# aleju/cat-generator

Hardware: AMD Instinct MI355X
Metric: images/sec per G+D step, G32up-c 32x32 RGB bs=128 per GPU (higher is better)
Workload: dtype f32

## Files before the change

### cat-generator_amd/csrc/common.h

```cpp
#pragma once
#include <hip/hip_runtime.h>
#include <algorithm>
#include <stdint.h>
#include <stdio.h>
#include <string.h>
#include "../../include/catgan.h"

namespace cg {

char* err_buf();
int fail(const char* fmt, ...);

inline hipStream_t S(void* s) { return reinterpret_cast<hipStream_t>(s); }

#define CG_HIP(call)                                                              \
    do {                                                                          \
        hipError_t e__ = (call);                                                  \
        if (e__ != hipSuccess)                                                    \
            return cg::fail("%s:%d %s -> %s", __FILE__, __LINE__, #call,          \
                            hipGetErrorString(e__));                              \
    } while (0)

#define CG_LAUNCH_CHECK()                                                         \
    do {                                                                          \
        hipError_t e__ = hipGetLastError();                                       \
        if (e__ != hipSuccess)                                                    \
            return cg::fail("%s:%d kernel launch -> %s", __FILE__, __LINE__,      \
                            hipGetErrorString(e__));                              \
    } while (0)

#define CG_REQUIRE(cond, ...)                                                     \
    do {                                                                          \
        if (!(cond)) return cg::fail(__VA_ARGS__);                                \
    } while (0)

constexpr int kNumCU = 256;

#ifndef CG_TIMING_PROBE
#define CG_TIMING_PROBE 0
#endif
#define CG_PROBE_HALF(fam, T) (((CG_TIMING_PROBE) & (fam)) ? ((T) + 1) / 2 : (T))
constexpr int kEwWgsPerCU = 4, kColReduceWgsPerCU = 1;

enum Opt {
    OPT_SKINNY, OPT_GEMM_BK32, OPT_WINO_BK, OPT_NN_TILE, OPT_TN_TILE, OPT_NN_SPLITS, OPT_TN_SPLITS,
    OPT_XCD_SWIZZLE, OPT_NN_GLDS, OPT_TN_GLDS, OPT_WINO_GLDS, OPT_PAD_SKIP, OPT_WINO3, OPT_WINO_DGRAD_FUSE, OPT_WINO_DGRAD_FUSE_LAUNCHES,
    OPT_WINO3_LAUNCHES, OPT_PACK_WIDE, OPT_SAMPLER_ATOMIC_LAUNCHES, OPT_COUNT
};
long opt(Opt o);
void opt_count(Opt o);

static inline int cdiv(long a, long b) { return (int)((a + b - 1) / b); }

constexpr size_t kColScratchBytes = 8u << 20;
void* col_scratch(hipStream_t stream);
hipStream_t queue_stream(hipStream_t ref, int cls, int slot);
int queue_class(hipStream_t ref, hipStream_t s);

constexpr int MAXG = 4;
constexpr int kMaxStridedGroups = 36;
template <typename T>
__device__ __forceinline__ T sel4(int i, T a, T b, T c, T d) { return i == 0 ? a : (i == 1 ? b : (i == 2 ? c : d)); }
__device__ __forceinline__ float4 ld4(const float* p) { return *reinterpret_cast<const float4*>(p); }
__device__ __forceinline__ float f4c(const float4& v, int i) { return i == 0 ? v.x : (i == 1 ? v.y : (i == 2 ? v.z : v.w)); }
template <typename T>
static inline void set4(T& p0, T& p1, T& p2, T& p3, const T* src, int n) {
    T* const dst[MAXG] = {&p0, &p1, &p2, &p3};
    for (int i = 0; i < MAXG; ++i) *dst[i] = (src && i < n) ? src[i] : nullptr;
}
__device__ __host__ __forceinline__ int phase_map(int a, int d, int pad) { return ((a + d - pad) >> 1) - ((a - pad) >> 1); }
static inline int phase_kp(int k, int pad) { return phase_map(0, k - 1, pad) + 1; }

struct WgradParts {
    const float* part;
    const float* bias_part;
    float* const* gw;
    float* const* gb;
    long gws;
    int ngroups, S, Cin, Cout, kH, kW, pad, ups;
    float scale;
};
int wgrad_finish(hipStream_t st, const WgradParts& w, bool defer);
void wgrad_discard_all();

constexpr int kSkinnyWgradBlocks = 512;
bool skinny_ok(int ngroups, int Cin, int Cout, int kH, int kW, int padH, int padW, int ups);
size_t skinny_wgrad_ws_bytes(int Cin, int Cout);
void skinny_valu_forward(hipStream_t st, const float* x, const float* w, const float* bias, float* y, int N, int H, int W, int Cin, int Cout);
void skinny_valu_wgrad(hipStream_t st, const float* x, const float* dy, float* part, float* bias_part, int N, int H, int W, int Cin, int Cout,
                       int blocks, long ppb);
bool skinny_mfma_ok(int Cin, int Cout, int H, int W);
int skinny_mfma_forward(hipStream_t st, const float* x, const float* w, const float* bias, float* y, int N, int H, int W, int Cin, int Cout);
int skinny_mfma_wgrad(hipStream_t st, const float* x, const float* dy, float* part, float* bias_part, int N, int H, int W, int Cin, int Cout,
                      int max_blocks);

bool head_wgrad_ok(int N, int T, int C, int Co);
int head_wgrad(hipStream_t st, const float* x, const float* dy, float* gw, float* gb, int N, int T, int C, int Co, float scale);
constexpr int kWino3UOffset = 9 * 64 * 64, kWino3UFloats = 16 * 64 * 64;
static inline bool wino3_layer(int Cout, int Cin, int kH, int kW) { return Cout == 64 && Cin == 64 && kH == 3 && kW == 3; }
bool wino3_geom_ok(int ngroups, int N, int H, int W, int Cin, int Cout, int kH, int kW, int padH, int padW, int ups);
int wino3_note_pack(hipStream_t st, int n, const float* const* w, float* const* wf, float* const* wb, const int* Cout, const int* Cin,
                    const int* kH, const int* kW, const int* wb_map);
int wino3_forward(hipStream_t st, int ngroups, const float* const* x, const float* const* wpk, const float* const* bias, float* const* y,
                  int N, int H, int W);

static inline int ew_grid(long n, int per_block = 256) {
    long b = (n + per_block - 1) / per_block;
    if (b < 1) b = 1;
    const long cap = (long)kNumCU * kEwWgsPerCU;
    if (b > cap) b = cap;
    return (int)b;
}

static inline bool al16(const void* p) { return ((uintptr_t)p & 15) == 0; }
template <class... P>
static inline bool vec_ok(long n, const P*... p) { return n % 4 == 0 && (al16(p) && ...); }

constexpr int tile_of_row_c(int l) {
    return ((l < 4 || (l >= 12 && l < 16) || (l >= 20 && l < 28)) ? 0 : 16) +
           ((l < 4 || (l >= 12 && l < 16) || (l >= 20 && l < 28)) ? (l < 4 ? l : (l < 16 ? l - 8 : l - 12)) : (l < 12 ? l - 4 : (l < 20 ? l - 8 : l - 16)));
}
__device__ __forceinline__ int tile_of_row(int l) {
    const bool ga = l < 4 || (l >= 12 && l < 16) || (l >= 20 && l < 28);
    const int rank = ga ? (l < 4 ? l : (l < 16 ? l - 8 : l - 12)) : (l < 12 ? l - 4 : (l < 20 ? l - 8 : l - 16));
    return (ga ? 0 : 16) + rank;
}
__device__ __forceinline__ void wino3_pack_item(const float* __restrict__ w, float* uf, float* ub, int idx) {
    constexpr int C = 64;
    const int co = idx / C, ci = idx % C;
    const float G[4][3] = {{1.f, 0.f, 0.f}, {.5f, .5f, .5f}, {.5f, -.5f, .5f}, {0.f, 0.f, 1.f}};
    for (int flip = 0; flip < 2; ++flip) {
        float* U = flip ? ub : uf;
        if (!U) continue;
        float g[3][3];
        for (int a = 0; a < 3; ++a)
            for (int b = 0; b < 3; ++b) g[a][b] = flip ? w[((long)ci * C + co) * 9 + (2 - a) * 3 + (2 - b)] : w[((long)co * C + ci) * 9 + a * 3 + b];
        float t[4][3];
        for (int i = 0; i < 4; ++i)
            for (int b = 0; b < 3; ++b) t[i][b] = G[i][0] * g[0][b] + G[i][1] * g[1][b] + G[i][2] * g[2][b];
        for (int i = 0; i < 4; ++i)
            for (int k = 0; k < 4; ++k)
                U[(((long)(i * 4 + k) * (C / 4) + ci / 4) * C + co) * 4 + (ci & 3)] = t[i][0] * G[k][0] + t[i][1] * G[k][1] + t[i][2] * G[k][2];
    }
}
__device__ __forceinline__ float u01(uint64_t seed, uint64_t ctr) {
    uint64_t z = seed + (ctr + 1) * 0x9E3779B97F4A7C15ull;
    z = (z ^ (z >> 30)) * 0xBF58476D1CE4E5B9ull;
    z = (z ^ (z >> 27)) * 0x94D049BB133111EBull;
    z = z ^ (z >> 31);
    return (float)(z >> 40) * (1.0f / 16777216.0f);
}
__device__ __forceinline__ float wave_sum(float v) {
#pragma unroll
    for (int off = 32; off > 0; off >>= 1) v += __shfl_down(v, off, 64);
    return v;
}
__device__ __forceinline__ double wave_sum(double v) {
#pragma unroll
    for (int off = 32; off > 0; off >>= 1) v += __shfl_down(v, off, 64);
    return v;
}

#ifndef CG_COL_HANDOVER
#define CG_COL_HANDOVER 3
#endif
__device__ __forceinline__ void st_agent(double* p, double v) {
#if CG_COL_HANDOVER == 4
    const unsigned long long old = __hip_atomic_exchange((unsigned long long*)p, (unsigned long long)__double_as_longlong(v),
                                                         __ATOMIC_RELAXED, __HIP_MEMORY_SCOPE_AGENT);
    asm volatile("" ::"v"(old));
#else
    __hip_atomic_store(p, v, __ATOMIC_RELAXED, __HIP_MEMORY_SCOPE_AGENT);
#endif
}
__device__ __forceinline__ double ld_agent(const double* p) {
#if CG_COL_HANDOVER == 4
    unsigned long long zero = 0ull;
    asm volatile("" : "+v"(zero));
    return __longlong_as_double((long long)__hip_atomic_fetch_or((unsigned long long*)const_cast<double*>(p), zero, __ATOMIC_RELAXED,
                                                                 __HIP_MEMORY_SCOPE_AGENT));
#else
    return __hip_atomic_load(const_cast<double*>(p), __ATOMIC_RELAXED, __HIP_MEMORY_SCOPE_AGENT);
#endif
}

__device__ __forceinline__ bool last_block_arrives(unsigned* counter, unsigned total) {
    __shared__ int last_flag;
#if CG_COL_HANDOVER == 0
    __threadfence();
#else
    asm volatile("s_waitcnt vmcnt(0)" ::: "memory");
#endif
    __syncthreads();
    if (threadIdx.x == 0) {
#if CG_COL_HANDOVER == 3
        __builtin_amdgcn_fence(__ATOMIC_RELEASE, "agent");
#endif
        const unsigned t = __hip_atomic_fetch_add(counter, 1u, __ATOMIC_RELAXED, __HIP_MEMORY_SCOPE_AGENT);
        last_flag = (t == total - 1) ? 1 : 0;
        if (last_flag) __hip_atomic_store(counter, 0u, __ATOMIC_RELAXED, __HIP_MEMORY_SCOPE_AGENT);
    }
    __syncthreads();
#if CG_COL_HANDOVER == 0
    if (last_flag) __threadfence();
#elif CG_COL_HANDOVER == 3
    if (last_flag) __builtin_amdgcn_fence(__ATOMIC_ACQUIRE, "agent");
#endif
    return last_flag != 0;
}

struct ColTree {
    int G, ngroups;
    unsigned* counters;
    double* part;
    double* grp;
    double* extra;
};
constexpr int kColTreeMaxGroups = 32;
static inline bool col_tree_layout(char* scr, long chunks, size_t nk, size_t nextra, ColTree& t) {
    t.G = (int)std::max<long>(16, (chunks + kColTreeMaxGroups - 1) / kColTreeMaxGroups);
    t.ngroups = (int)((chunks + t.G - 1) / t.G);
    t.counters = (unsigned*)scr;
    t.part = (double*)(scr + 256);
    t.grp = t.part + (size_t)chunks * nk;
    t.extra = t.grp + (size_t)t.ngroups * nk;
    return 256 + sizeof(double) * ((size_t)chunks * nk + (size_t)t.ngroups * nk + nextra) <= kColScratchBytes;
}

__device__ __forceinline__ void col_sum_rows(const double* rows, int nrows, int nk, double* out) {
    for (int k = threadIdx.x; k < nk; k += blockDim.x) {
        double t = 0.0;
        int y = 0;
        for (; y + 16 <= nrows; y += 16) {
            double v[16];
#pragma unroll
            for (int j = 0; j < 16; ++j) v[j] = ld_agent(&rows[(size_t)(y + j) * nk + k]);
#pragma unroll
            for (int j = 0; j < 16; ++j) t += v[j];
        }
        for (; y < nrows; ++y) t += ld_agent(&rows[(size_t)y * nk + k]);
        st_agent(&out[k], t);
    }
}

__device__ __forceinline__ bool col_tree_finish(const ColTree& t, int chunk, int chunks, unsigned blocks_per_chunk, int nk, double* sums) {
    const int g = chunk / t.G;
    const int in_group = min(t.G, chunks - g * t.G);
    if (!last_block_arrives(t.counters + 1 + g, (unsigned)in_group * blocks_per_chunk)) return false;
    col_sum_rows(t.part + (size_t)g * t.G * nk, in_group, nk, t.grp + (size_t)g * nk);
    if (!last_block_arrives(t.counters, (unsigned)t.ngroups)) return false;
    col_sum_rows(t.grp, t.ngroups, nk, sums);
    return true;
}

__device__ __forceinline__ double block_sum_256(double v, double* sh ) {
    v = wave_sum(v);
    const int lane = threadIdx.x & 63, wave = threadIdx.x >> 6;
    if (lane == 0) sh[wave] = v;
    __syncthreads();
    double r = 0.0;
    if (threadIdx.x == 0) r = sh[0] + sh[1] + sh[2] + sh[3];
    __syncthreads();
    return r;
}

#define CG_GRID_STRIDE(i, n) \
    for (long i = blockIdx.x * (long)blockDim.x + threadIdx.x; i < (n); i += (long)gridDim.x * blockDim.x)

template <int VW> struct Vec;
template <> struct Vec<1> {
    typedef float T;
    static __device__ __forceinline__ T zero() { return 0.f; }
    static __device__ __forceinline__ T ld(const float* p) { return *p; }
    static __device__ __forceinline__ void st(float* p, T v) { *p = v; }
    static __device__ __forceinline__ float dot(T a, T b) { return a * b; }
    static __device__ __forceinline__ void fma(T& acc, float w, T g) { acc += w * g; }
    T v;
    __device__ __forceinline__ float& operator[](int) { return v; }
    __device__ __forceinline__ float operator[](int) const { return v; }
    static __device__ __forceinline__ Vec load(const float* p, long i) { return Vec{p[i]}; }
    __device__ __forceinline__ void store(float* p, long i) const { p[i] = v; }
    static __device__ __forceinline__ Vec ldc(const float* p, int c) { return Vec{p[c]}; }
};
template <> struct Vec<4> {
    typedef float4 T;
    static __device__ __forceinline__ T zero() { return make_float4(0.f, 0.f, 0.f, 0.f); }
    static __device__ __forceinline__ T ld(const float* p) { return *reinterpret_cast<const float4*>(p); }
    static __device__ __forceinline__ void st(float* p, T v) { *reinterpret_cast<float4*>(p) = v; }
    static __device__ __forceinline__ float dot(T a, T b) { return ((a.x * b.x + a.y * b.y) + a.z * b.z) + a.w * b.w; }
    static __device__ __forceinline__ void fma(T& acc, float w, T g) { acc.x += w * g.x; acc.y += w * g.y; acc.z += w * g.z; acc.w += w * g.w; }
    T v;
    __device__ __forceinline__ float& operator[](int k) { return (&v.x)[k]; }
    __device__ __forceinline__ float operator[](int k) const { return (&v.x)[k]; }
    static __device__ __forceinline__ Vec load(const float* p, long i) { return Vec{ld(p + 4 * i)}; }
    __device__ __forceinline__ void store(float* p, long i) const { st(p + 4 * i, v); }
    static __device__ __forceinline__ Vec ldc(const float* p, int c) { return Vec{make_float4(p[4 * c], p[4 * c + 1], p[4 * c + 2], p[4 * c + 3])}; }
};

__device__ __forceinline__ bool act_passes(int act, float x) { return act == 0 || (act == 1 ? x > 0.f : x >= 0.f); }
__device__ __forceinline__ float act(int act, float v, float a) { return act_passes(act, v) ? v : a * v; }
__device__ __forceinline__ float dact(int act, float x, float d, float a) { return act_passes(act, x) ? d : a * d; }
__device__ __forceinline__ float slope_term(float x, float d) { return x <= 0.f ? x * d : 0.f; }
template <int VW>
__device__ __forceinline__ void slope_acc(float& s, const Vec<VW>& x, const Vec<VW>& d) {
    if constexpr (VW == 1) {
        if (x[0] <= 0.f) s = fmaf(x[0], d[0], s);
    } else {
        float t = slope_term(x[0], d[0]);
#pragma unroll
        for (int k = 1; k < VW; ++k) t += slope_term(x[k], d[k]);
        s += t;
    }
}
template <int VW>
__device__ __forceinline__ void prelu_bwd_walk(const float* x, const float* dy, float a, float* dx, long n, double* partial) {
    __shared__ double sh[4];
    float s = 0.f;
    CG_GRID_STRIDE(i, n) {
        const Vec<VW> v = Vec<VW>::load(x, i), g = Vec<VW>::load(dy, i);
        Vec<VW> o;
#pragma unroll
        for (int k = 0; k < VW; ++k) o[k] = dact(1, v[k], g[k], a);
        o.store(dx, i);
        slope_acc(s, v, g);
    }
    if (!partial) return;
    const double t = block_sum_256((double)s, sh);
    if (threadIdx.x == 0) *partial = t;
}
__device__ __forceinline__ double partials_sum_256(const double* part, int nparts) {
    __shared__ double sh[4];
    double s = 0.0;
    for (int i = threadIdx.x; i < nparts; i += 256) s += part[i];
    return block_sum_256(s, sh);
}
__device__ __forceinline__ float bn_xhat(float x, float m, float s) { return (x - m) * s; }
__device__ __forceinline__ float bn_norm(float x, float m, float s, float g, float b) { return bn_xhat(x, m, s) * g + b; }
__device__ __forceinline__ float bn_dx(float x, float dy, float g, float m, float s, float m1, float m2) {
    return g * s * (dy - m1 - bn_xhat(x, m, s) * m2);
}
__device__ __forceinline__ float augment_noise(uint64_t seed, uint64_t ctr) {
    unsigned S = 0;
#pragma unroll
    for (int k = 0; k < 3; ++k) {
        uint64_t z = seed + (ctr + k + 1) * 0x9E3779B97F4A7C15ull;
        z = (z ^ (z >> 30)) * 0xBF58476D1CE4E5B9ull;
        z = (z ^ (z >> 27)) * 0x94D049BB133111EBull;
        z = z ^ (z >> 31);
        S += (unsigned)(z & 0xFFFF) + (unsigned)((z >> 16) & 0xFFFF) + (unsigned)((z >> 32) & 0xFFFF) + (unsigned)(z >> 48);
    }
// ... 13 lines not shown
```

### cat-generator_amd/csrc/ops.hip

```cpp
#include "common.h"
#include <stdarg.h>
#include <stdlib.h>
#include <algorithm>

namespace cg {
char* err_buf() {
    static thread_local char buf[512] = {0};
    return buf;
}
int fail(const char* fmt, ...) {
    va_list ap;
    va_start(ap, fmt);
    vsnprintf(err_buf(), 512, fmt, ap);
    va_end(ap);
    return 1;
}

namespace {
struct OptDef { const char* name; long dflt; };
const OptDef kOptDefs[OPT_COUNT] = {
    {"CG_SKINNY", 1}, {"CG_GEMM_BK32", 1}, {"CG_WINO_BK", 0}, {"CG_NN_TILE", 0}, {"CG_TN_TILE", 0}, {"CG_NN_SPLITS", 0}, {"CG_TN_SPLITS", 0},
    {"CG_XCD_SWIZZLE", 7}, {"CG_NN_GLDS", 1}, {"CG_TN_GLDS", 1}, {"CG_WINO_GLDS", 1}, {"CG_PAD_SKIP", 20}, {"CG_WINO3", 1},
    {"CG_WINO_DGRAD_FUSE", 1}, {"CG_WINO_DGRAD_FUSE_LAUNCHES", 0}, {"CG_WINO3_LAUNCHES", 0}, {"CG_PACK_WIDE", 1},
    {"CG_SAMPLER_ATOMIC_LAUNCHES", 0},
};
long g_opt_val[OPT_COUNT];
int g_opt_state[OPT_COUNT];
}

}
#include <chrono>
#include <mutex>
#include <unordered_map>
#include <vector>
namespace cg {
void* col_scratch(hipStream_t stream) {
    constexpr int kPool = 8, kReserve = 4;
    static std::unordered_map<hipStream_t, void*> blocks;
    static std::vector<void*> pool;
    static std::mutex mu;
    std::lock_guard<std::mutex> lk(mu);
    auto it = blocks.find(stream);
    if (it != blocks.end()) return it->second;
    hipStreamCaptureStatus st = hipStreamCaptureStatusNone;
    const bool capturing = stream && hipStreamIsCapturing(stream, &st) == hipSuccess && st != hipStreamCaptureStatusNone;
    if (capturing && pool.empty()) {
        cg::fail("column reduce: no scratch block left for a stream first used inside a graph capture (run one pass on it before cg_graph_begin)");
        return nullptr;
    }
    if (!capturing && (int)pool.size() <= kReserve) {
        char* p = nullptr;
        hipStreamCaptureMode mode = hipStreamCaptureModeRelaxed;
        (void)hipThreadExchangeStreamCaptureMode(&mode);
        const bool ok = hipMalloc((void**)&p, kColScratchBytes * kPool) == hipSuccess &&
                        hipMemsetAsync(p, 0, kColScratchBytes * kPool, stream) == hipSuccess &&
                        hipStreamSynchronize(stream) == hipSuccess;
        (void)hipThreadExchangeStreamCaptureMode(&mode);
        if (!ok) {
            (void)hipGetLastError();
            if (pool.empty()) { cg::fail("column reduce: cannot allocate %zu bytes of scratch", kColScratchBytes * kPool); return nullptr; }
        } else
            for (int i = kPool - 1; i >= 0; --i) pool.insert(pool.begin(), p + (size_t)i * kColScratchBytes);
    }
    void* blk = pool.back();
    pool.pop_back();
    blocks[stream] = blk;
    return blk;
}
namespace {
__global__ void queue_probe_spin_k(unsigned long long ticks, int* sink) {
    const unsigned long long t0 = wall_clock64();
    while (wall_clock64() - t0 < ticks) { }
    if (ticks == ~0ull) *sink = 1;
}
struct QueuePool {
    std::vector<hipStream_t> s;
    std::unordered_map<hipStream_t, std::vector<int>> cls;
    std::mutex mu;
};
QueuePool& qpool() { static QueuePool p; return p; }
constexpr int kQueuePool = 24;

double probe_pair(hipStream_t a, hipStream_t b, bool both, unsigned long long ticks) {
    (void)hipStreamSynchronize(a);
    if (both) (void)hipStreamSynchronize(b);
    const auto t0 = std::chrono::steady_clock::now();
    hipLaunchKernelGGL(queue_probe_spin_k, dim3(1), dim3(64), 0, a, ticks, (int*)nullptr);
    if (both) hipLaunchKernelGGL(queue_probe_spin_k, dim3(1), dim3(64), 0, b, ticks, (int*)nullptr);
    (void)hipStreamSynchronize(a);
    if (both) (void)hipStreamSynchronize(b);
    return std::chrono::duration<double, std::milli>(std::chrono::steady_clock::now() - t0).count();
}
bool same_queue(hipStream_t a, hipStream_t b) {
    const unsigned long long ticks = 30000;
    int votes = 0;
    for (int r = 0; r < 3; ++r) {
        const double one = probe_pair(a, a, false, ticks), two = probe_pair(a, b, true, ticks);
        if (two > 1.6 * one) ++votes;
    }
    return votes >= 2;
}
}

int queue_classify(hipStream_t ref) {
    QueuePool& p = qpool();
    hipStreamCaptureStatus st = hipStreamCaptureStatusNone;
    if (ref && hipStreamIsCapturing(ref, &st) == hipSuccess && st != hipStreamCaptureStatusNone)
        return cg::fail("queue_stream: a stream's hardware queue cannot be probed inside a graph capture (run one pass on it before cg_graph_begin)");
    while ((int)p.s.size() < kQueuePool) {
        hipStream_t q;
        if (hipStreamCreateWithFlags(&q, hipStreamNonBlocking) != hipSuccess) return cg::fail("queue_stream: hipStreamCreate failed");
        p.s.push_back(q);
    }
    std::vector<int> c(p.s.size(), -1);
    std::vector<hipStream_t> rep;
    for (size_t i = 0; i < p.s.size(); ++i) {
        if (same_queue(ref, p.s[i])) { c[i] = 0; continue; }
        for (size_t k = 0; k < rep.size() && c[i] < 0; ++k)
            if (same_queue(rep[k], p.s[i])) c[i] = (int)k + 1;
        if (c[i] < 0) { rep.push_back(p.s[i]); c[i] = (int)rep.size(); }
    }
    (void)hipGetLastError();
    p.cls[ref] = c;
    return 0;
}

hipStream_t queue_stream(hipStream_t ref, int cls, int slot) {
    QueuePool& p = qpool();
    std::lock_guard<std::mutex> lk(p.mu);
    if (!p.cls.count(ref) && queue_classify(ref)) return nullptr;
    const std::vector<int>& c = p.cls[ref];
    int nclass = 0;
    for (int v : c) nclass = std::max(nclass, v + 1);
    if (nclass < 2) {
        static bool warned = false;
        if (!warned) { warned = true; fprintf(stderr, "cg: the hardware-queue probe found one queue only - side streams are plain pool streams (overlap not guaranteed)\n"); }
        return p.s[(size_t)((cls & 3) * (kQueuePool / 4) + slot % (kQueuePool / 4)) % p.s.size()];
    }
    cls = cls % nclass;
    int seen = 0;
    hipStream_t last = nullptr;
    for (size_t i = 0; i < c.size(); ++i)
        if (c[i] == cls) { last = p.s[i]; if (seen++ == slot) return p.s[i]; }
    if (last) return last;
    cg::fail("queue_stream: no pool stream on hardware queue class %d", cls);
    return nullptr;
}

int queue_class(hipStream_t ref, hipStream_t s) {
    if (s == ref) return 0;
    QueuePool& p = qpool();
    std::lock_guard<std::mutex> lk(p.mu);
    auto it = p.cls.find(ref);
    if (it == p.cls.end()) return -1;
    for (size_t i = 0; i < p.s.size(); ++i) if (p.s[i] == s) return it->second[i];
    return -1;
}

unsigned long g_opt_epoch = 1;
long opt(Opt o) {
    if (g_opt_state[o] == 0) {
        const char* e = getenv(kOptDefs[o].name);
        g_opt_val[o] = e ? atol(e) : kOptDefs[o].dflt;
        g_opt_state[o] = 1;
    }
    return g_opt_val[o];
}
void opt_count(Opt o) { opt(o); ++g_opt_val[o]; }
}

namespace {
using cg::block_sum_256;
using cg::last_block_arrives;
using cg::wave_sum;

#define GRID_STRIDE(i, n) CG_GRID_STRIDE(i, n)

enum { CS_RGB = 0, CS_Y = 1, CS_YUV = 2, CS_HSL = 3 };
__device__ __forceinline__ void store_colorspace(float* dst, long i, float r, float g, float b, int cs) {
#pragma clang fp contract(off)
    if (cs == CS_RGB) { dst[3 * i] = r; dst[3 * i + 1] = g; dst[3 * i + 2] = b; }
    else if (cs == CS_Y) {
        const float t0 = 0.21f * r, t1 = 0.72f * g, t2 = 0.07f * b;
        dst[i] = (t0 + t1) + t2;
    } else if (cs == CS_YUV) {
        const float y0 = 0.299f * r, y1 = 0.587f * g, y2 = 0.114f * b;
        const float u0 = -0.14713f * r, u1 = 0.28886f * g, u2 = 0.436f * b;
        const float v0 = 0.615f * r, v1 = 0.51499f * g, v2 = 0.10001f * b;
        dst[3 * i] = (y0 + y1) + y2; dst[3 * i + 1] = (u0 - u1) + u2; dst[3 * i + 2] = (v0 - v1) - v2;
    } else {
        const float mx = fmaxf(r, fmaxf(g, b)), mn = fminf(r, fminf(g, b));
        const float sum = mx + mn, l = __fdiv_rn(sum, 2.f);
        float h = 0.f, s = 0.f;
        if (mx != mn) {
            const float d = mx - mn;
            s = l > 0.5f ? __fdiv_rn(d, (2.f - mx) - mn) : __fdiv_rn(d, sum);
            if (mx == r) h = __fdiv_rn(g - b, d) + (g < b ? 6.f : 0.f);
            else if (mx == g) h = __fdiv_rn(b - r, d) + 2.f;
            else h = __fdiv_rn(r - g, d) + 4.f;
            h = __fdiv_rn(h, 6.f);
        }
        dst[3 * i] = h; dst[3 * i + 1] = s; dst[3 * i + 2] = l;
    }
}
__device__ __forceinline__ float hsl_hue(float p, float q, float t) {
#pragma clang fp contract(off)
    const float sixth = (float)(1.0 / 6.0), two_thirds = (float)(2.0 / 3.0);
    if (t < 0.f) t += 1.f;
    if (t > 1.f) t -= 1.f;
    if (t < sixth) { const float a = (q - p) * 6.f, m = a * t; return p + m; }
    if (t < 0.5f) return q;
    if (t < two_thirds) { const float a = (q - p) * (two_thirds - t), m = a * 6.f; return p + m; }
    return p;
}
__device__ __forceinline__ void colorspace_to_rgb(float a, float b, float c, int cs, float* rgb) {
#pragma clang fp contract(off)
    if (cs == CS_YUV) {
        const float rv = 1.13983f * c, gu = 0.39465f * b, gv = 0.58060f * c, bu = 2.03211f * b;
        rgb[0] = a + rv; rgb[1] = (a - gu) - gv; rgb[2] = a + bu;
    } else {
        const float h = a, s = b, l = c;
        if (s == 0.f) { rgb[0] = l; rgb[1] = l; rgb[2] = l; return; }
        const float third = (float)(1.0 / 3.0);
        const float ls = l * s;
        const float q = l < 0.5f ? l * (1.f + s) : (l + s) - ls;
        const float p = 2.f * l - q;
        rgb[0] = hsl_hue(p, q, h + third); rgb[1] = hsl_hue(p, q, h); rgb[2] = hsl_hue(p, q, h - third);
    }
}
__global__ void colorspace_convert_k(const float* src, float* dst, long npix, int from, int to) {
    GRID_STRIDE(i, npix) {
        const float a = src[3 * i], b = src[3 * i + 1], c = src[3 * i + 2];
        if (from == CS_RGB) store_colorspace(dst, i, a, b, c, to);
        else {
            float rgb[3];
            colorspace_to_rgb(a, b, c, from, rgb);
            dst[3 * i] = rgb[0]; dst[3 * i + 1] = rgb[1]; dst[3 * i + 2] = rgb[2];
        }
    }
}
__global__ void images_u8_to_f32_k(const unsigned char* __restrict__ src, float* __restrict__ dst, long npix, int cs) {
#pragma clang fp contract(off)
    GRID_STRIDE(i, npix) {
        const float r = __fdiv_rn((float)src[3 * i], 255.f), g = __fdiv_rn((float)src[3 * i + 1], 255.f), b = __fdiv_rn((float)src[3 * i + 2], 255.f);
        store_colorspace(dst, i, r, g, b, cs);
    }
}

__device__ __forceinline__ float scale_axis(const float* w, int base, int Ls, int Ld, int d) {
#pragma clang fp contract(off)
#define s(k) w[(k) - base]
    if (Ld == Ls) return s(d);
    if (Ld > Ls) {
        if (d == Ld - 1 || Ls == 1) return s(Ls == 1 ? 0 : Ls - 1);
        const float scale = __fdiv_rn((float)(Ls - 1), (float)(Ld - 1));
        float sf = (float)d * scale;
        const int si = (int)sf;
        sf -= (float)si;
        const float a = (1.f - sf) * s(si), b = sf * s(si + 1);
        return a + b;
    }
    const float scale = __fdiv_rn((float)Ls, (float)Ld);
    float f0 = (float)d * scale;
    int i0 = (int)f0;
    f0 -= (float)i0;
    if (d == 0) { i0 = 0; f0 = 0.f; }
    float f1 = (float)(d + 1) * scale;
    const int i1 = (int)f1;
    f1 -= (float)i1;
    float acc = (1.f - f0) * s(i0), n = 1.f - f0;
    for (int si = i0 + 1; si < i1; ++si) { acc += s(si); n += 1.f; }
    if (i1 < Ls) { const float t = f1 * s(i1); acc += t; n += f1; }
    return __fdiv_rn(acc, n);
#undef s
}
__device__ __forceinline__ void scale_pixel(const unsigned char* __restrict__ im, float* __restrict__ dst, long i, int ox, int oy, int Hs, int Ws,
                                            int Hd, int Wd, int cs) {
#pragma clang fp contract(off)
    int y0 = oy, y1 = oy;
    if (Hd < Hs) {
        const float scale = __fdiv_rn((float)Hs, (float)Hd);
        y0 = oy == 0 ? 0 : (int)((float)oy * scale);
        y1 = min(Hs - 1, (int)((float)(oy + 1) * scale));
    } else if (Hd > Hs) {
        const float scale = __fdiv_rn((float)(Hs - 1), (float)(Hd - 1));
        y0 = (oy == Hd - 1 || Hs == 1) ? Hs - 1 : (int)((float)oy * scale);
        y1 = min(Hs - 1, y0 + 1);
    }
    float rgb[3];
    for (int c = 0; c < 3; ++c) {
        float col[8];
        for (int y = y0; y <= y1 && y - y0 < 8; ++y) {
            int x0 = ox, x1 = ox;
            if (Wd < Ws) {
                const float sc = __fdiv_rn((float)Ws, (float)Wd);
                x0 = ox == 0 ? 0 : (int)((float)ox * sc);
                x1 = min(Ws - 1, (int)((float)(ox + 1) * sc));
            } else if (Wd > Ws) {
                const float sc = __fdiv_rn((float)(Ws - 1), (float)(Wd - 1));
                x0 = (ox == Wd - 1 || Ws == 1) ? Ws - 1 : (int)((float)ox * sc);
                x1 = min(Ws - 1, x0 + 1);
            }
            float row[8];
            for (int x = x0; x <= x1 && x - x0 < 8; ++x) row[x - x0] = __fdiv_rn((float)im[((long)y * Ws + x) * 3 + c], 255.f);
            col[y - y0] = scale_axis(row, x0, Ws, Wd, ox);
        }
        rgb[c] = scale_axis(col, y0, Hs, Hd, oy);
    }
    store_colorspace(dst, i, rgb[0], rgb[1], rgb[2], cs);
}
__device__ __forceinline__ void store_zero_pixel(float* dst, long i, int cs) {
    if (cs == CS_Y) dst[i] = 0.f;
    else { dst[3 * i] = 0.f; dst[3 * i + 1] = 0.f; dst[3 * i + 2] = 0.f; }
}
__global__ void images_u8_scale_k(const unsigned char* __restrict__ src, float* __restrict__ dst, int N, int Hs, int Ws, int Hd, int Wd, int cs) {
    const long total = (long)N * Hd * Wd;
    GRID_STRIDE(i, total) {
        const int ox = (int)(i % Wd), oy = (int)((i / Wd) % Hd);
        const long n = i / ((long)Wd * Hd);
        scale_pixel(src + n * (long)Hs * Ws * 3, dst, i, ox, oy, Hs, Ws, Hd, Wd, cs);
    }
}
__global__ void images_u8_gather_scale_k(const unsigned char* __restrict__ set, long M, const int32_t* __restrict__ idx, float* __restrict__ dst,
                                         int N, int Hs, int Ws, int Hd, int Wd, int cs) {
    const long total = (long)N * Hd * Wd;
    GRID_STRIDE(i, total) {
        const int ox = (int)(i % Wd), oy = (int)((i / Wd) % Hd);
// ... 1605 lines not shown
```

### cat-generator_amd/csrc/wino3.hip

```cpp
#include "common.h"

namespace {

typedef float f32x16 __attribute__((ext_vector_type(16)));
typedef unsigned int u32x4 __attribute__((ext_vector_type(4)));
typedef float f32x4 __attribute__((ext_vector_type(4)));
constexpr int C = 64;
constexpr int PLD = 68;
constexpr int PW = 18, PH = 10;
constexpr int kUFloats = cg::kWino3UFloats;

using cg::ld4;
__device__ __forceinline__ float4 bufld4(__amdgpu_buffer_rsrc_t r, unsigned voff, int soff) {
    const u32x4 v = __builtin_amdgcn_raw_buffer_load_b128(r, voff, soff, 0);
    const f32x4 f = __builtin_bit_cast(f32x4, v);
    return make_float4(f.x, f.y, f.z, f.w);
}

struct PackJobs { const float* w[8]; float* uf[8]; float* ub[8]; int n; };
__global__ void wino3_pack_k(PackJobs jobs) {
    cg::wino3_pack_item(jobs.w[blockIdx.y], jobs.uf[blockIdx.y], jobs.ub[blockIdx.y], blockIdx.x * 256 + threadIdx.x);
}

using cg::tile_of_row;
using cg::tile_of_row_c;

template <int XI>
__device__ __forceinline__ void wino_row(const float* P, int tyl, int txl, int h, __amdgpu_buffer_rsrc_t rsU, unsigned uvoff, f32x16 (&T)[2]) {
    constexpr int I1 = XI == 0 ? 0 : (XI == 2 ? 2 : 1), I2 = XI == 0 ? 2 : (XI == 1 ? 2 : (XI == 2 ? 1 : 3));
    constexpr bool PLUS = XI == 1;
    const float* pt = P + ((2 * tyl) * PW + 2 * txl) * PLD;
    const float* r1 = pt + I1 * PW * PLD + ((h ^ ((tyl + (I1 >> 1)) & 1)) << 2);
    const float* r2 = pt + I2 * PW * PLD + ((h ^ ((tyl + (I2 >> 1)) & 1)) << 2);
    f32x16 acc[4];
#pragma unroll
    for (int k = 0; k < 4; ++k)
#pragma unroll
        for (int r = 0; r < 16; ++r) acc[k][r] = 0.f;
#pragma unroll 2
    for (int s = 0; s < CG_PROBE_HALF(8, 8); ++s) {
        float4 e[4];
#pragma unroll
        for (int c = 0; c < 4; ++c) {
            const float4 d1 = ld4(r1 + c * PLD + 8 * s), d2 = ld4(r2 + c * PLD + 8 * s);
            e[c].x = PLUS ? d1.x + d2.x : d1.x - d2.x; e[c].y = PLUS ? d1.y + d2.y : d1.y - d2.y;
            e[c].z = PLUS ? d1.z + d2.z : d1.z - d2.z; e[c].w = PLUS ? d1.w + d2.w : d1.w - d2.w;
        }
        float4 v[4], ua[4];
#pragma unroll
        for (int nu = 0; nu < 4; ++nu) {
            constexpr int J1[4] = {0, 1, 2, 1}, J2[4] = {2, 2, 1, 3};
            const float4 a = e[J1[nu]], b = e[J2[nu]];
            if (nu == 1) { v[nu].x = a.x + b.x; v[nu].y = a.y + b.y; v[nu].z = a.z + b.z; v[nu].w = a.w + b.w; }
            else { v[nu].x = a.x - b.x; v[nu].y = a.y - b.y; v[nu].z = a.z - b.z; v[nu].w = a.w - b.w; }
            ua[nu] = bufld4(rsU, uvoff, (((XI * 4 + nu) * 16 + 2 * s) * C) * 16);
        }
#define CG_W3_MF(comp) \
    _Pragma("unroll") for (int nu = 0; nu < 4; ++nu) acc[nu] = __builtin_amdgcn_mfma_f32_32x32x2f32(v[nu].comp, ua[nu].comp, acc[nu], 0, 0, 0);
        CG_W3_MF(x) CG_W3_MF(y) CG_W3_MF(z) CG_W3_MF(w)
#undef CG_W3_MF
    }
#pragma unroll
    for (int r = 0; r < 16; ++r) { T[0][r] = (acc[0][r] + acc[1][r]) + acc[2][r]; T[1][r] = (acc[1][r] - acc[2][r]) - acc[3][r]; }
}

struct W3Args {
    const float* x[4]; const float* u[4]; const float* bias[4]; float* y[4];
    int N, H, W;
};

__global__ __launch_bounds__(512, 2) void wino3_fused_k(W3Args a) {
    __shared__ __attribute__((aligned(16))) float P[PH * PW * PLD];
    const int tid = threadIdx.x, lane = tid & 63, wave = __builtin_amdgcn_readfirstlane(tid >> 6);
    const int j = lane & 31, h = lane >> 5;
    const int xi = wave & 3, nt = wave >> 2;
    const int grp = blockIdx.y;
    const float* __restrict__ x = a.x[grp];
    const float* __restrict__ U = a.u[grp];
    float* __restrict__ y = a.y[grp];
    const int H = a.H, W = a.W;
    const int bxn = W >> 4, byn = H >> 3;
    int b = blockIdx.x;
    const int bx = b % bxn; b /= bxn;
    const int by = b % byn;
    const int n = b / byn;
    const int y0 = by * 8, x0 = bx * 16;

    {
        const __amdgpu_buffer_rsrc_t rsx = __builtin_amdgcn_make_buffer_rsrc((void*)(x + (long)n * H * W * C), 0, (unsigned)(H * W * C * 4), 0x00020000);
        const int q = tid & 15;
        int pix = tid >> 4, pr = pix / PW, pc = pix - pr * PW;
#pragma unroll
        for (int it = 0; it < (PH * PW + 31) / 32; ++it) {
            const int iy = y0 - 1 + pr, ix = x0 - 1 + pc;
            const bool in = iy >= 0 && iy < H && ix >= 0 && ix < W;
            const unsigned voff = in ? (unsigned)(((iy * W + ix) * C + q * 4) * 4) : 0x80000000u;
            const float4 v = bufld4(rsx, voff, 0);
            if (pix < PH * PW) *reinterpret_cast<float4*>(P + pix * PLD + ((q ^ ((pr >> 1) & 1)) << 2)) = v;
            pix += 32; pr += 1; pc += 14;
            if (pc >= PW) { pc -= PW; pr += 1; }
        }
    }
    __syncthreads();

    const int tl = tile_of_row(j), tyl = tl >> 3, txl = tl & 7;
    const __amdgpu_buffer_rsrc_t rsU = __builtin_amdgcn_make_buffer_rsrc((void*)U, 0, kUFloats * 4, 0x00020000);
    const unsigned uvoff = (unsigned)(h * C + nt * 32 + j) * 16u;
    f32x16 T[2];
    if (xi == 0) wino_row<0>(P, tyl, txl, h, rsU, uvoff, T);
    else if (xi == 1) wino_row<1>(P, tyl, txl, h, rsU, uvoff, T);
    else if (xi == 2) wino_row<2>(P, tyl, txl, h, rsU, uvoff, T);
    else wino_row<3>(P, tyl, txl, h, rsU, uvoff, T);

    __syncthreads();
    float* X = P + nt * 6 * 1024;
#pragma unroll
    for (int r = 0; r < 16; ++r) {
        const int k = r * 64 + lane;
        if (xi == 1) { X[0 * 1024 + k] = T[0][r]; X[5 * 1024 + k] = T[1][r]; }
        if (xi == 2) { X[1 * 1024 + k] = T[0][r]; X[3 * 1024 + k] = T[1][r]; }
        if (xi == 0) X[2 * 1024 + k] = T[1][r];
        if (xi == 3) X[4 * 1024 + k] = T[0][r];
    }
    __syncthreads();
    const int oa = xi >> 1, ob = xi & 1;
    const float* bias = a.bias[grp];
    const float bco = bias ? bias[nt * 32 + j] : 0.f;
    const __amdgpu_buffer_rsrc_t rsy = __builtin_amdgcn_make_buffer_rsrc((void*)(y + (long)n * H * W * C), 0, (unsigned)(H * W * C * 4), 0x00020000);
    const int lane_base = (((y0 + oa) * W + x0 + ob) * C + nt * 32 + j) * 4;
    const int rowb = 2 * W * C * 4, colb = 2 * C * 4;
#pragma unroll
    for (int r = 0; r < 16; ++r) {
        const int k = r * 64 + lane;
        float v;
        if (xi == 0) v = (T[0][r] + X[0 * 1024 + k]) + X[1 * 1024 + k];
        else if (xi == 1) v = (X[2 * 1024 + k] + T[1][r]) + X[3 * 1024 + k];
        else if (xi == 2) v = (X[0 * 1024 + k] - T[0][r]) - X[4 * 1024 + k];
        else v = (X[5 * 1024 + k] - X[3 * 1024 + k]) - T[1][r];
        const int row0 = (r & 3) + 8 * (r >> 2);
        const int t0 = tile_of_row_c(row0), t1 = tile_of_row_c(row0 + 4);
        const int off0 = (t0 >> 3) * rowb + (t0 & 7) * colb, off1 = (t1 >> 3) * rowb + (t1 & 7) * colb;
        __builtin_amdgcn_raw_buffer_store_b32(__float_as_uint(v + bco), rsy, lane_base + (h ? off1 : off0), 0, 0);
    }
}

}

namespace cg {

bool wino3_geom_ok(int ngroups, int N, int H, int W, int Cin, int Cout, int kH, int kW, int padH, int padW, int ups) {
    if (!(ups == 0 && kH == 3 && kW == 3 && padH == 1 && padW == 1 && Cin == C && Cout == C && H % 8 == 0 && W % 16 == 0)) return false;
    if (ngroups < 1 || ngroups > 4) return false;
    const long v = opt(OPT_WINO3);
    const bool full = (long)ngroups * N * (H / 8) * (W / 16) >= 2L * kNumCU;
    return v == 2 || (v == 1 && full);
}

int wino3_note_pack(hipStream_t st, int n, const float* const* w, float* const* wf, float* const* wb, const int* Cout, const int* Cin,
                    const int* kH, const int* kW, const int* wb_map) {
    PackJobs jobs;
    jobs.n = 0;
    auto flush = [&]() {
        if (jobs.n) hipLaunchKernelGGL(wino3_pack_k, dim3(C * C / 256, jobs.n), dim3(256), 0, st, jobs);
        jobs.n = 0;
    };
    for (int i = 0; i < n; ++i) {
        if (!wino3_layer(Cout[i], Cin[i], kH[i], kW[i]) || (wb_map && wb_map[i])) continue;
        jobs.w[jobs.n] = w[i];
        jobs.uf[jobs.n] = wf[i] ? wf[i] + kWino3UOffset : nullptr;
        jobs.ub[jobs.n] = wb[i] ? wb[i] + kWino3UOffset : nullptr;
        if (++jobs.n == 8) flush();
    }
    flush();
    CG_LAUNCH_CHECK();
    return 0;
}

int wino3_forward(hipStream_t st, int ngroups, const float* const* x, const float* const* wpk, const float* const* bias, float* const* y,
                  int N, int H, int W) {
    W3Args a;
    memset(&a, 0, sizeof(a));
    for (int g = 0; g < ngroups; ++g) {
        if (!wpk[g] || !x[g] || !y[g] || (uintptr_t)x[g] % 16 || (uintptr_t)wpk[g] % 16) return 0;
        a.x[g] = x[g]; a.u[g] = wpk[g] + kWino3UOffset; a.bias[g] = bias ? bias[g] : nullptr; a.y[g] = y[g];
    }
    a.N = N; a.H = H; a.W = W;
    hipLaunchKernelGGL(wino3_fused_k, dim3((unsigned)(N * (H / 8) * (W / 16)), ngroups), dim3(512), 0, st, a);
    if (hipGetLastError() != hipSuccess) { cg::fail("wino3_forward: launch failed"); return -1; }
    opt_count(OPT_WINO3_LAUNCHES);
    return 1;
}

}
```

Before: 23620.

## Make Winograd 3x3 conv kernel persistent with prefetch of next input patch

```diff
diff --git a/cat-generator_amd/csrc/common.h b/cat-generator_amd/csrc/common.h
--- a/cat-generator_amd/csrc/common.h
+++ b/cat-generator_amd/csrc/common.h
@@ -45,7 +45,7 @@
 enum Opt {
     OPT_SKINNY, OPT_GEMM_BK32, OPT_WINO_BK, OPT_NN_TILE, OPT_TN_TILE, OPT_NN_SPLITS, OPT_TN_SPLITS,
     OPT_XCD_SWIZZLE, OPT_NN_GLDS, OPT_TN_GLDS, OPT_WINO_GLDS, OPT_PAD_SKIP, OPT_WINO3, OPT_WINO_DGRAD_FUSE, OPT_WINO_DGRAD_FUSE_LAUNCHES,
-    OPT_WINO3_LAUNCHES, OPT_PACK_WIDE, OPT_SAMPLER_ATOMIC_LAUNCHES, OPT_COUNT
+    OPT_WINO3_LAUNCHES, OPT_PACK_WIDE, OPT_SAMPLER_ATOMIC_LAUNCHES, OPT_WINO3_RESIDENT, OPT_WINO3_WGS, OPT_COUNT
 };
 long opt(Opt o);
 void opt_count(Opt o);
diff --git a/cat-generator_amd/csrc/ops.hip b/cat-generator_amd/csrc/ops.hip
--- a/cat-generator_amd/csrc/ops.hip
+++ b/cat-generator_amd/csrc/ops.hip
@@ -22,7 +22,7 @@
     {"CG_SKINNY", 1}, {"CG_GEMM_BK32", 1}, {"CG_WINO_BK", 0}, {"CG_NN_TILE", 0}, {"CG_TN_TILE", 0}, {"CG_NN_SPLITS", 0}, {"CG_TN_SPLITS", 0},
     {"CG_XCD_SWIZZLE", 7}, {"CG_NN_GLDS", 1}, {"CG_TN_GLDS", 1}, {"CG_WINO_GLDS", 1}, {"CG_PAD_SKIP", 20}, {"CG_WINO3", 1},
     {"CG_WINO_DGRAD_FUSE", 1}, {"CG_WINO_DGRAD_FUSE_LAUNCHES", 0}, {"CG_WINO3_LAUNCHES", 0}, {"CG_PACK_WIDE", 1},
-    {"CG_SAMPLER_ATOMIC_LAUNCHES", 0},
+    {"CG_SAMPLER_ATOMIC_LAUNCHES", 0}, {"CG_WINO3_RESIDENT", 1}, {"CG_WINO3_WGS", 0},
 };
 long g_opt_val[OPT_COUNT];
 int g_opt_state[OPT_COUNT];
diff --git a/cat-generator_amd/csrc/wino3.hip b/cat-generator_amd/csrc/wino3.hip
--- a/cat-generator_amd/csrc/wino3.hip
+++ b/cat-generator_amd/csrc/wino3.hip
@@ -25,7 +25,7 @@
 using cg::tile_of_row;
 using cg::tile_of_row_c;
 
-template <int XI>
+template <int XI, bool PK>
 __device__ __forceinline__ void wino_row(const float* P, int tyl, int txl, int h, __amdgpu_buffer_rsrc_t rsU, unsigned uvoff, f32x16 (&T)[2]) {
     constexpr int I1 = XI == 0 ? 0 : (XI == 2 ? 2 : 1), I2 = XI == 0 ? 2 : (XI == 1 ? 2 : (XI == 2 ? 1 : 3));
     constexpr bool PLUS = XI == 1;
@@ -39,21 +39,36 @@
         for (int r = 0; r < 16; ++r) acc[k][r] = 0.f;
 #pragma unroll 2
     for (int s = 0; s < CG_PROBE_HALF(8, 8); ++s) {
-        float4 e[4];
-#pragma unroll
-        for (int c = 0; c < 4; ++c) {
-            const float4 d1 = ld4(r1 + c * PLD + 8 * s), d2 = ld4(r2 + c * PLD + 8 * s);
-            e[c].x = PLUS ? d1.x + d2.x : d1.x - d2.x; e[c].y = PLUS ? d1.y + d2.y : d1.y - d2.y;
-            e[c].z = PLUS ? d1.z + d2.z : d1.z - d2.z; e[c].w = PLUS ? d1.w + d2.w : d1.w - d2.w;
-        }
         float4 v[4], ua[4];
-#pragma unroll
-        for (int nu = 0; nu < 4; ++nu) {
-            constexpr int J1[4] = {0, 1, 2, 1}, J2[4] = {2, 2, 1, 3};
-            const float4 a = e[J1[nu]], b = e[J2[nu]];
-            if (nu == 1) { v[nu].x = a.x + b.x; v[nu].y = a.y + b.y; v[nu].z = a.z + b.z; v[nu].w = a.w + b.w; }
-            else { v[nu].x = a.x - b.x; v[nu].y = a.y - b.y; v[nu].z = a.z - b.z; v[nu].w = a.w - b.w; }
-            ua[nu] = bufld4(rsU, uvoff, (((XI * 4 + nu) * 16 + 2 * s) * C) * 16);
+        constexpr int J1[4] = {0, 1, 2, 1}, J2[4] = {2, 2, 1, 3};
+        if (PK) {
+            f32x4 e[4];
+#pragma unroll
+            for (int c = 0; c < 4; ++c) {
+                const f32x4 d1 = *reinterpret_cast<const f32x4*>(r1 + c * PLD + 8 * s), d2 = *reinterpret_cast<const f32x4*>(r2 + c * PLD + 8 * s);
+                e[c] = PLUS ? d1 + d2 : d1 - d2;
+            }
+#pragma unroll
+            for (int nu = 0; nu < 4; ++nu) {
+                const f32x4 t = nu == 1 ? e[J1[nu]] + e[J2[nu]] : e[J1[nu]] - e[J2[nu]];
+                v[nu] = make_float4(t.x, t.y, t.z, t.w);
+                ua[nu] = bufld4(rsU, uvoff, (((XI * 4 + nu) * 16 + 2 * s) * C) * 16);
+            }
+        } else {
+            float4 e[4];
+#pragma unroll
+            for (int c = 0; c < 4; ++c) {
+                const float4 d1 = ld4(r1 + c * PLD + 8 * s), d2 = ld4(r2 + c * PLD + 8 * s);
+                e[c].x = PLUS ? d1.x + d2.x : d1.x - d2.x; e[c].y = PLUS ? d1.y + d2.y : d1.y - d2.y;
+                e[c].z = PLUS ? d1.z + d2.z : d1.z - d2.z; e[c].w = PLUS ? d1.w + d2.w : d1.w - d2.w;
+            }
+#pragma unroll
+            for (int nu = 0; nu < 4; ++nu) {
+                const float4 a = e[J1[nu]], b = e[J2[nu]];
+                if (nu == 1) { v[nu].x = a.x + b.x; v[nu].y = a.y + b.y; v[nu].z = a.z + b.z; v[nu].w = a.w + b.w; }
+                else { v[nu].x = a.x - b.x; v[nu].y = a.y - b.y; v[nu].z = a.z - b.z; v[nu].w = a.w - b.w; }
+                ua[nu] = bufld4(rsU, uvoff, (((XI * 4 + nu) * 16 + 2 * s) * C) * 16);
+            }
         }
 #define CG_W3_MF(comp) \
     _Pragma("unroll") for (int nu = 0; nu < 4; ++nu) acc[nu] = __builtin_amdgcn_mfma_f32_32x32x2f32(v[nu].comp, ua[nu].comp, acc[nu], 0, 0, 0);
@@ -69,7 +84,7 @@
     int N, H, W;
 };
 
-__global__ __launch_bounds__(512, 2) void wino3_fused_k(W3Args a) {
+__global__ __launch_bounds__(512, 2) void wino3_oneblock_k(W3Args a) {
     __shared__ __attribute__((aligned(16))) float P[PH * PW * PLD];
     const int tid = threadIdx.x, lane = tid & 63, wave = __builtin_amdgcn_readfirstlane(tid >> 6);
     const int j = lane & 31, h = lane >> 5;
@@ -107,10 +122,10 @@
     const __amdgpu_buffer_rsrc_t rsU = __builtin_amdgcn_make_buffer_rsrc((void*)U, 0, kUFloats * 4, 0x00020000);
     const unsigned uvoff = (unsigned)(h * C + nt * 32 + j) * 16u;
     f32x16 T[2];
-    if (xi == 0) wino_row<0>(P, tyl, txl, h, rsU, uvoff, T);
-    else if (xi == 1) wino_row<1>(P, tyl, txl, h, rsU, uvoff, T);
-    else if (xi == 2) wino_row<2>(P, tyl, txl, h, rsU, uvoff, T);
-    else wino_row<3>(P, tyl, txl, h, rsU, uvoff, T);
+    if (xi == 0) wino_row<0, false>(P, tyl, txl, h, rsU, uvoff, T);
+    else if (xi == 1) wino_row<1, false>(P, tyl, txl, h, rsU, uvoff, T);
+    else if (xi == 2) wino_row<2, false>(P, tyl, txl, h, rsU, uvoff, T);
+    else wino_row<3, false>(P, tyl, txl, h, rsU, uvoff, T);
 
     __syncthreads();
     float* X = P + nt * 6 * 1024;
@@ -141,6 +156,119 @@
         const int t0 = tile_of_row_c(row0), t1 = tile_of_row_c(row0 + 4);
         const int off0 = (t0 >> 3) * rowb + (t0 & 7) * colb, off1 = (t1 >> 3) * rowb + (t1 & 7) * colb;
         __builtin_amdgcn_raw_buffer_store_b32(__float_as_uint(v + bco), rsy, lane_base + (h ? off1 : off0), 0, 0);
+    }
+}
+
+constexpr int kPatchIts = (PH * PW + 31) / 32;
+constexpr int kResidentWgs = 2 * cg::kNumCU;
+
+__device__ __forceinline__ int fresh(int v) { asm volatile("" : "+v"(v)); return v; }
+
+__device__ __forceinline__ void patch_load(float4 (&pf)[kPatchIts], const float* x, int b, bool valid, int H, int W, int tid) {
+    const int bxn = W >> 4, byn = H >> 3;
+    const int bx = b % bxn, by = (b / bxn) % byn, n = b / (bxn * byn);
+    const __amdgpu_buffer_rsrc_t rsx = __builtin_amdgcn_make_buffer_rsrc((void*)(x + (long)n * H * W * C), 0, (unsigned)(H * W * C * 4), 0x00020000);
+    const int q = tid & 15, pix0 = tid >> 4;
+#pragma unroll
+    for (int it = 0; it < kPatchIts; ++it) {
+        const int pix = pix0 + 32 * it, pr = pix / PW, pc = pix - pr * PW;
+        const int iy = by * 8 - 1 + pr, ix = bx * 16 - 1 + pc;
+        const bool in = valid & ((unsigned)iy < (unsigned)H) & ((unsigned)ix < (unsigned)W);
+        pf[it] = bufld4(rsx, in ? (unsigned)(((iy * W + ix) * C + q * 4) * 4) : 0x80000000u, 0);
+    }
+}
+__device__ __forceinline__ void patch_store(float* P, const float4 (&pf)[kPatchIts], int tid) {
+    const int q = tid & 15, pix0 = tid >> 4;
+#pragma unroll
+    for (int it = 0; it < kPatchIts; ++it) {
+        const int pix = pix0 + 32 * it, pr = pix / PW;
+        if (pix < PH * PW) *reinterpret_cast<float4*>(P + pix * PLD + ((q ^ ((pr >> 1) & 1)) << 2)) = pf[it];
+    }
+}
+template <int XI>
+__device__ __forceinline__ void publish(float* X, int lane, const f32x16 (&T)[2]) {
+#pragma unroll
+    for (int r = 0; r < 16; ++r) {
+        const int k = r * 64 + lane;
+        if (XI == 1) { X[0 * 1024 + k] = T[0][r]; X[5 * 1024 + k] = T[1][r]; }
+        if (XI == 2) { X[1 * 1024 + k] = T[0][r]; X[3 * 1024 + k] = T[1][r]; }
+        if (XI == 0) X[2 * 1024 + k] = T[1][r];
+        if (XI == 3) X[4 * 1024 + k] = T[0][r];
+    }
+}
+template <int XI>
+__device__ __forceinline__ void finish(const float* X, int lane, const f32x16 (&T)[2], float (&v)[16]) {
+#pragma unroll
+    for (int r = 0; r < 16; ++r) {
+        const int k = r * 64 + lane;
+        if (XI == 0) v[r] = (T[0][r] + X[0 * 1024 + k]) + X[1 * 1024 + k];
+        else if (XI == 1) v[r] = (X[2 * 1024 + k] + T[1][r]) + X[3 * 1024 + k];
+        else if (XI == 2) v[r] = (X[0 * 1024 + k] - T[0][r]) - X[4 * 1024 + k];
+        else v[r] = (X[5 * 1024 + k] - X[3 * 1024 + k]) - T[1][r];
+    }
+}
+
+__global__ __launch_bounds__(512, 4) void wino3_fused_k(W3Args a) {
+    __shared__ __attribute__((aligned(16))) float P[12 * 1024];
+    const int wave = __builtin_amdgcn_readfirstlane(threadIdx.x >> 6);
+    const int xi = wave & 3, nt = wave >> 2;
+    const int grp = blockIdx.y;
+    const float* __restrict__ x = a.x[grp];
+    const float* __restrict__ bias = a.bias[grp];
+    float* __restrict__ y = a.y[grp];
+    const int H = a.H, W = a.W;
+    const int bxn = W >> 4, byn = H >> 3, nblocks = a.N * byn * bxn;
+    const __amdgpu_buffer_rsrc_t rsU = __builtin_amdgcn_make_buffer_rsrc((void*)a.u[grp], 0, kUFloats * 4, 0x00020000);
+    float* X = P + nt * 6 * 1024;
+    float4 pf[kPatchIts];
+    int b = blockIdx.x;
+    patch_load(pf, x, b, true, H, W, fresh(threadIdx.x));
+    patch_store(P, pf, fresh(threadIdx.x));
+    for (;;) {
+        __syncthreads();
+        f32x16 T[2];
+        {
+            const int tid = fresh(threadIdx.x), j = tid & 31, h = (tid >> 5) & 1;
+            const int tl = tile_of_row(j), tyl = tl >> 3, txl = tl & 7;
+            const unsigned uvoff = (unsigned)(h * C + nt * 32 + j) * 16u;
+            if (xi == 0) wino_row<0, true>(P, tyl, txl, h, rsU, uvoff, T);
+            else if (xi == 1) wino_row<1, true>(P, tyl, txl, h, rsU, uvoff, T);
+            else if (xi == 2) wino_row<2, true>(P, tyl, txl, h, rsU, uvoff, T);
+            else wino_row<3, true>(P, tyl, txl, h, rsU, uvoff, T);
+        }
+        const int bn = b + (int)gridDim.x;
+        const bool more = bn < nblocks;
+        const float bco = bias ? bias[nt * 32 + (fresh(threadIdx.x) & 31)] : 0.f;
+        patch_load(pf, x, more ? bn : b, more, H, W, fresh(threadIdx.x));
+        __syncthreads();
+        const int tid = fresh(threadIdx.x), lane = tid & 63, j = tid & 31, h = (tid >> 5) & 1;
+        if (xi == 0) publish<0>(X, lane, T);
+        else if (xi == 1) publish<1>(X, lane, T);
+        else if (xi == 2) publish<2>(X, lane, T);
+        else publish<3>(X, lane, T);
+        __syncthreads();
+        float v[16];
+        if (xi == 0) finish<0>(X, lane, T, v);
+        else if (xi == 1) finish<1>(X, lane, T, v);
+        else if (xi == 2) finish<2>(X, lane, T, v);
+        else finish<3>(X, lane, T, v);
+        if (more) {
+            __syncthreads();
+            patch_store(P, pf, fresh(threadIdx.x));
+        }
+        const int bx = b % bxn, by = (b / bxn) % byn, n = b / (bxn * byn);
+        const __amdgpu_buffer_rsrc_t rsy = __builtin_amdgcn_make_buffer_rsrc((void*)(y + (long)n * H * W * C), 0, (unsigned)(H * W * C * 4), 0x00020000);
+        const int lane_base = (((by * 8 + (xi >> 1)) * W + bx * 16 + (xi & 1)) * C + nt * 32 + j) * 4;
+        const int rowb = 2 * W * C * 4, colb = 2 * C * 4;
+#pragma unroll
+        for (int r = 0; r < 16; ++r) {
+            const int row0 = (r & 3) + 8 * (r >> 2);
+            const int t0 = tile_of_row_c(row0), t1 = tile_of_row_c(row0 + 4);
+            const int off0 = (t0 >> 3) * rowb + (t0 & 7) * colb, off1 = (t1 >> 3) * rowb + (t1 & 7) * colb;
+            __builtin_amdgcn_raw_buffer_store_b32(__float_as_uint(v[r] + bco), rsy, lane_base + (h ? off1 : off0), 0, 0);
+        }
+        if (!more) break;
+        b = bn;
     }
 }
 
@@ -185,7 +313,14 @@
         a.x[g] = x[g]; a.u[g] = wpk[g] + kWino3UOffset; a.bias[g] = bias ? bias[g] : nullptr; a.y[g] = y[g];
     }
     a.N = N; a.H = H; a.W = W;
-    hipLaunchKernelGGL(wino3_fused_k, dim3((unsigned)(N * (H / 8) * (W / 16)), ngroups), dim3(512), 0, st, a);
+    const int blocks = N * (H / 8) * (W / 16);
+    if (opt(OPT_WINO3_RESIDENT) == 0)
+        hipLaunchKernelGGL(wino3_oneblock_k, dim3((unsigned)blocks, ngroups), dim3(512), 0, st, a);
+    else {
+        const long cap = opt(OPT_WINO3_WGS);
+        const int wgs = (int)std::min<long>(blocks, cap > 0 ? cap : std::max(1, kResidentWgs / ngroups));
+        hipLaunchKernelGGL(wino3_fused_k, dim3((unsigned)wgs, ngroups), dim3(512), 0, st, a);
+    }
     if (hipGetLastError() != hipSuccess) { cg::fail("wino3_forward: launch failed"); return -1; }
     opt_count(OPT_WINO3_LAUNCHES);
     return 1;
```

New measurement: 23600. Within noise of the previous version (-0.1%).
